# rueberger/MJHMC

Hardware: AMD Instinct MI355X
Metric: particle-steps/sec (ndims x nparticles x L) (higher is better)
Workload: dtype f64 state (ProductOfT: around the f32 matrix-core force)

## Files before the change

### mjhmc_amd/csrc/dense_pot64_kernels.hpp

```cpp
#pragma once
#ifndef __HIPCC_RTC__
#include <hip/hip_runtime.h>
#endif
#include <stdint.h>

#include "dense_pot.hpp"
#include "dense_pot_tile.hpp"
#include "group_form.hpp"

namespace mjhmc {

template <int NB>
struct DVecN;
template <>
struct DVecN<1> {
  using type = double;
};
template <>
struct DVecN<2> {
  using type = __attribute__((ext_vector_type(2))) double;
};
template <>
struct DVecN<4> {
  using type = __attribute__((ext_vector_type(4))) double;
};
template <int NB>
__device__ __forceinline__ double dget(const typename DVecN<NB>::type& v, int r) {
  if constexpr (NB == 1) return v;
  else return v[r];
}
template <int NB>
__device__ __forceinline__ void dset(typename DVecN<NB>::type& v, int r, double x) {
  if constexpr (NB == 1) v = x;
  else v[r] = x;
}

template <int NB>
__device__ __forceinline__ int q_off(int q) { return NB * ((q & 3) + 8 * (q >> 2)); }
template <int NB>
__device__ __forceinline__ const double* lane_row(const double* base, int64_t p, int w, int h) {
  return base + (size_t)p * (128 * NB) + 32 * NB * w + 4 * NB * h;
}
template <int NB>
__device__ __forceinline__ double* lane_row(double* base, int64_t p, int w, int h) {
  return base + (size_t)p * (128 * NB) + 32 * NB * w + 4 * NB * h;
}
template <int NB>
__device__ __forceinline__ typename DVecN<NB>::type dv_load(const double* lrow, int q) {
  return *reinterpret_cast<const typename DVecN<NB>::type*>(lrow + q_off<NB>(q));
}
template <int NB>
__device__ __forceinline__ void dv_store(double* lrow, int q, const typename DVecN<NB>::type& v) {
  *reinterpret_cast<typename DVecN<NB>::type*>(lrow + q_off<NB>(q)) = v;
}

template <int NB>
constexpr int kA64 = NB == 4 ? 8 : 16;
template <int NB>
using AReg64 = AReg<NB, kA64<NB>>;

constexpr int kPark = 8;
template <int NB>
struct Shared64 {
  Shared<NB> s;
  double red64[4][kP];
  double zn[128 * NB];
  f32x4 park[kPark / 2][256];
};

using uvec4 = __attribute__((ext_vector_type(4))) unsigned;
using f64x2 = __attribute__((ext_vector_type(2))) double;

template <int NB>
struct PieceOf {
  using type = uvec4;
};
template <>
struct PieceOf<1> {
  using type = unsigned long long;
};
__device__ __forceinline__ int here(int lane_const) {
  asm volatile("" : "+v"(lane_const));
  return lane_const;
}
template <int NB>
struct Stage {
  using P = typename PieceOf<NB>::type;
  static constexpr int PB = sizeof(P);
  static constexpr int RB = 1024 * NB;
  static constexpr int RP = RB / PB;
  static constexpr int K = 32 * RP / 256;
  static constexpr int KB = K < 16 ? K : 16;
};
__device__ __forceinline__ unsigned stage_addr(int row, int piece, int pb, int rb) {
  return (unsigned)(row * rb + ((piece ^ (row & 15)) * pb));
}
template <int NB>
__device__ __forceinline__ void stage_rows_in(const double* rows, int64_t p, char* img) {
  using S = Stage<NB>;
  using P = typename S::P;
  const int t = here(threadIdx.x);
#pragma unroll 1
  for (int i0 = 0; i0 < S::K; i0 += S::KB) {
    P buf[S::KB];
#pragma unroll
    for (int i = 0; i < S::KB; ++i) {
      const int k = (i0 + i) * 256 + t, row = k / S::RP, piece = k % S::RP;
      const int64_t pr = __shfl((long long)p, row);
      buf[i] = *reinterpret_cast<const P*>(reinterpret_cast<const char*>(rows) + (size_t)pr * S::RB + (size_t)piece * S::PB);
    }
#pragma unroll
    for (int i = 0; i < S::KB; ++i) {
      const int k = (i0 + i) * 256 + t, row = k / S::RP, piece = k % S::RP;
      *reinterpret_cast<P*>(img + stage_addr(row, piece, S::PB, S::RB)) = buf[i];
    }
  }
}
template <int NB>
__device__ __forceinline__ void stage_rows_out(double* rows, int64_t p, const char* img) {
  using S = Stage<NB>;
  using P = typename S::P;
  const int t = here(threadIdx.x);
#pragma unroll 1
  for (int i0 = 0; i0 < S::K; i0 += S::KB) {
#pragma unroll
    for (int i = 0; i < S::KB; ++i) {
      const int k = (i0 + i) * 256 + t, row = k / S::RP, piece = k % S::RP;
      const int64_t pr = __shfl((long long)p, row);
      *reinterpret_cast<P*>(reinterpret_cast<char*>(rows) + (size_t)pr * S::RB + (size_t)piece * S::PB) =
          *reinterpret_cast<const P*>(img + stage_addr(row, piece, S::PB, S::RB));
    }
  }
}
template <int NB>
__device__ __forceinline__ typename DVecN<NB>::type stage_get(const char* img, int w, int c, int h, int q) {
  using S = Stage<NB>;
  const int first = (8 * NB * (32 * w + acc_row(q, h))) / S::PB;
  if constexpr (NB == 4) {
    const f64x2 lo = *reinterpret_cast<const f64x2*>(img + stage_addr(c, first, S::PB, S::RB));
    const f64x2 hi = *reinterpret_cast<const f64x2*>(img + stage_addr(c, first + 1, S::PB, S::RB));
    typename DVecN<4>::type v;
    v[0] = lo[0];
    v[1] = lo[1];
    v[2] = hi[0];
    v[3] = hi[1];
    return v;
  } else {
    return *reinterpret_cast<const typename DVecN<NB>::type*>(img + stage_addr(c, first, S::PB, S::RB));
  }
}
template <int NB>
__device__ __forceinline__ void stage_put(char* img, int w, int c, int h, int q, const typename DVecN<NB>::type& v) {
  using S = Stage<NB>;
  const int first = (8 * NB * (32 * w + acc_row(q, h))) / S::PB;
  if constexpr (NB == 4) {
    f64x2 lo, hi;
    lo[0] = v[0];
    lo[1] = v[1];
    hi[0] = v[2];
    hi[1] = v[3];
    *reinterpret_cast<f64x2*>(img + stage_addr(c, first, S::PB, S::RB)) = lo;
    *reinterpret_cast<f64x2*>(img + stage_addr(c, first + 1, S::PB, S::RB)) = hi;
  } else {
    *reinterpret_cast<typename DVecN<NB>::type*>(img + stage_addr(c, first, S::PB, S::RB)) = v;
  }
}
template <int NB>
__device__ __forceinline__ char* stage_image(Shared<NB>& s) {
  static_assert(sizeof(s.pub) == 32 * Stage<NB>::RB, "the staging image is the two B-operand images");
  return reinterpret_cast<char*>(&s.pub[0][0]);
}

template <int NB>
struct VTile {
  double b[NB][16];
};

template <int NB, int NKICK>
__device__ __forceinline__ void kick_drift_pass(const Tile<NB>& g, VTile<NB>& v, VTile<NB>& x, double c, double eps,
                                                PubWave<NB>* pub0, int w, int lane) {
#pragma unroll
  for (int q4 = 0; q4 < 4; ++q4) {
    f32x4 px[NB];
#pragma unroll
    for (int qq = 0; qq < 4; ++qq) {
      const int q = 4 * q4 + qq;
#pragma unroll
      for (int r = 0; r < NB; ++r) {
        const double t = c * (double)g.b[r][q];
        double vv = v.b[r][q];
        vv = vv + t;
        if constexpr (NKICK == 2) vv = vv + t;
        v.b[r][q] = vv;
        const double xx = x.b[r][q] + eps * vv;
        x.b[r][q] = xx;
        px[r][qq] = (float)xx;
      }
    }
#pragma unroll
    for (int r = 0; r < NB; ++r) pub0[w].v[r][q4][lane] = px[r];
    __builtin_amdgcn_sched_barrier(0);
  }
}

template <int NB>
__device__ __forceinline__ double closing_kick(const Tile<NB>& g, VTile<NB>& v, double c) {
  double s = 0.0;
#pragma unroll
  for (int q = 0; q < 16; ++q)
#pragma unroll
    for (int r = 0; r < NB; ++r) {
      const double vv = v.b[r][q] + c * (double)g.b[r][q];
      v.b[r][q] = vv;
      s = s + vv * vv;
    }
  return s;
}

template <int NB, class SH>
__device__ __forceinline__ double column_sum(SH& sh, int w, int c, int h, double part) {
  const double both = swap32_sum(part);
  if (h == 0) sh.red64[w][c] = both;
  __syncthreads();
  const double tot = sh.red64[0][c] + sh.red64[1][c] + sh.red64[2][c] + sh.red64[3][c];
  __syncthreads();
  return tot;
}

template <int NB>
__device__ __forceinline__ void staged_start(Shared<NB>& s, const double* xin, const double* vin, const double* gin, int64_t p,
                                             int w, int c, int h, Tile<NB>& g, VTile<NB>& v, VTile<NB>& x, bool neg) {
  char* img = stage_image<NB>(s);
  c = here(c), w = here(w), h = here(h);
  stage_rows_in<NB>(xin, p, img);
  __syncthreads();
#pragma unroll
  for (int q = 0; q < 16; ++q) {
    const typename DVecN<NB>::type xx = stage_get<NB>(img, w, c, h, q);
#pragma unroll
    for (int r = 0; r < NB; ++r) x.b[r][q] = dget<NB>(xx, r);
  }
  __syncthreads();
  stage_rows_in<NB>(gin, p, img);
  __syncthreads();
#pragma unroll
  for (int q = 0; q < 16; ++q) {
    const typename DVecN<NB>::type gg = stage_get<NB>(img, w, c, h, q);
#pragma unroll
    for (int r = 0; r < NB; ++r) g.b[r][q] = (float)dget<NB>(gg, r);
  }
  __syncthreads();
  stage_rows_in<NB>(vin, p, img);
  __syncthreads();
#pragma unroll
  for (int q = 0; q < 16; ++q) {
    const typename DVecN<NB>::type vv = stage_get<NB>(img, w, c, h, q);
#pragma unroll
    for (int r = 0; r < NB; ++r) v.b[r][q] = neg ? -dget<NB>(vv, r) : dget<NB>(vv, r);
  }
  __syncthreads();
}

template <int NB>
__device__ __forceinline__ void staged_end_x(Shared<NB>& s, double* xout, int64_t p, int w, int c, int h, const VTile<NB>& x) {
  char* img = stage_image<NB>(s);
  c = here(c), w = here(w), h = here(h);
#pragma unroll
  for (int q = 0; q < 16; ++q) {
    typename DVecN<NB>::type xx;
#pragma unroll
    for (int r = 0; r < NB; ++r) dset<NB>(xx, r, x.b[r][q]);
    stage_put<NB>(img, w, c, h, q, xx);
  }
  __syncthreads();
  stage_rows_out<NB>(xout, p, img);
  __syncthreads();
}
template <int NB>
__device__ __forceinline__ void staged_end_vg(Shared<NB>& s, double* vout, double* gout, int64_t p, int w, int c, int h,
                                              const VTile<NB>& v, const Tile<NB>& g) {
  using DV = typename DVecN<NB>::type;
  char* img = stage_image<NB>(s);
  c = here(c), w = here(w), h = here(h);
#pragma unroll
  for (int q = 0; q < 16; ++q) {
    DV vv;
#pragma unroll
    for (int r = 0; r < NB; ++r) dset<NB>(vv, r, v.b[r][q]);
    stage_put<NB>(img, w, c, h, q, vv);
  }
  __syncthreads();
  stage_rows_out<NB>(vout, p, img);
  __syncthreads();
#pragma unroll
  for (int q = 0; q < 16; ++q) {
    DV gg;
#pragma unroll
    for (int r = 0; r < NB; ++r) dset<NB>(gg, r, (double)g.b[r][q]);
    stage_put<NB>(img, w, c, h, q, gg);
  }
  __syncthreads();
  stage_rows_out<NB>(gout, p, img);
  __syncthreads();
}

template <int NB, class XP>
__device__ __forceinline__ double pot64_trajectory(const PotModel& mdl, const XP& xp, AReg64<NB>& ar, Shared64<NB>& sh, int w, int c, int h,
                                                   int lane, Tile<NB>& g, VTile<NB>& v, VTile<NB>& x, int L, double eps,
                                                   double chalf, float* ex) {
  PubWave<NB>* pub0 = sh.s.pub[0];
  kick_drift_pass<NB, 1>(g, v, x, chalf, eps, pub0, w, lane);
  for (int s = 0; s < L; ++s) {
    [[maybe_unused]] const int stamp_slot = s;
    POT_STAMP(0);
    if constexpr (NB == 4) {
#pragma unroll
      for (int k = 0; k < kPark / 2; ++k) {
        f64x2 two;
        two[0] = v.b[NB - 1][15 - 2 * k];
        two[1] = v.b[NB - 1][14 - 2 * k];
        sh.park[k][threadIdx.x] = __builtin_bit_cast(f32x4, two);
      }
    }
    pot_gradient_published<NB>(mdl, xp, ar, sh.s, w, c, h, lane, g, s == L - 1, ex, s);
    if constexpr (NB == 4) {
#pragma unroll
      for (int k = 0; k < kPark / 2; ++k) {
        const f64x2 two = __builtin_bit_cast(f64x2, sh.park[k][threadIdx.x]);
        v.b[NB - 1][15 - 2 * k] = two[0];
        v.b[NB - 1][14 - 2 * k] = two[1];
      }
#pragma unroll
      for (int r = 0; r < NB; ++r)
#pragma unroll
        for (int q = 0; q < 16; ++q) use_here(v.b[r][q]);
    }
    POT_STAMP(6);
    if (s < L - 1) kick_drift_pass<NB, 2>(g, v, x, chalf, eps, pub0, w, lane);
    POT_STAMP(7);
  }
  const double part = closing_kick<NB>(g, v, chalf);
  return column_sum<NB>(sh, w, c, h, part) / 2.0;
}


template <int NB>
struct Finish64Shared {
  struct {
    int move[kP];
  } s;
  double red64[4][kP];
  double zn[128 * NB];
};

template <int NB, bool REPLAY, int MODE, bool FIX, class SH>
__device__ __forceinline__ void pot64_finish(const Pot64JumpArgs& a, SH& sh, int64_t p, bool alive, size_t roff, int w, int c,
                                             int h, const VTile<NB>& v, const Tile<NB>& g) {
  using DV = typename DVecN<NB>::type;
  const double* xin = a.X_in + roff;
  const double* vin = a.V_in + roff;
  const double* gin = a.G_in + roff;
  double* xo = a.X_out + roff;
  double* vo = a.V_out + roff;
  double* go = a.G_out + roff;
  const int mv = sh.s.move[c];
  const int k = mv & 3;
  bool take, flip, refresh;
  if constexpr (MODE == kModeControl) {
    const bool accept = k & 1, fl = k & 2;
    take = accept;
    flip = accept != fl;
    refresh = (mv & 4) != 0;
  } else {
    take = k == 0;
    flip = (MODE == kModeCT && k == 0) || k == 1;
    refresh = k == 2;
  }
  const bool tile_refreshes = __ballot(refresh) != 0ull;
  if (!FIX || !take) {
#pragma unroll
    for (int q = 0; q < 16; ++q) {
      DV gg;
      if (take) {
        if constexpr (!FIX) {
          DV vv;
#pragma unroll
          for (int r = 0; r < NB; ++r) {
            dset<NB>(vv, r, flip ? -v.b[r][q] : v.b[r][q]);
            dset<NB>(gg, r, (double)g.b[r][q]);
          }
          dv_store<NB>(vo, q, vv);
        }
      } else {
        gg = dv_load<NB>(gin, q);
        dv_store<NB>(xo, q, dv_load<NB>(xin, q));
      }
      dv_store<NB>(go, q, gg);
    }
  }
  double s2 = 0.0;
  if (!take || (REPLAY && refresh)) {
    const double* vsrc = take ? (const double*)vo : vin;
    const bool fl2 = flip && !take;
    const double* nrow = REPLAY ? lane_row<NB>(a.noise, alive ? p : 0, w, h) : nullptr;
#pragma unroll 1
    for (int q = 0; q < 16; ++q) {
      DV vv = dv_load<NB>(vsrc, q);
      if (fl2) vv = -vv;
      if constexpr (REPLAY) {
        if (refresh) {
          const DV z = dv_load<NB>(nrow, q);
#pragma unroll
          for (int r = 0; r < NB; ++r) {
            const double t = dget<NB>(vv, r) * a.r_keep + dget<NB>(z, r) * a.r_mix;
            dset<NB>(vv, r, t);
            s2 = s2 + t * t;
          }
        }
      }
      dv_store<NB>(vo, q, vv);
    }
  }
  if constexpr (!REPLAY) {
    unsigned cols = (unsigned)(__ballot(refresh) & 0xFFFFFFFFull);
    while (cols) {
      const int c0 = __ffs((int)cols) - 1;
      cols &= cols - 1;
      const int64_t p0 = __shfl((long long)p, c0);
      column_normals<NB, double>(a.key, (uint32_t)(a.first_pid + (p0 < a.N ? p0 : 0)), a.D, sh.zn);
      __syncthreads();
      if (c == c0) {
        const double* zrow = sh.zn + 32 * NB * w + 4 * NB * h;
#pragma unroll 1
        for (int q = 0; q < 16; ++q) {
          DV vv = dv_load<NB>(vo, q);
          const DV z = *reinterpret_cast<const DV*>(zrow + q_off<NB>(q));
#pragma unroll
          for (int r = 0; r < NB; ++r) {
            const double t = dget<NB>(vv, r) * a.r_keep + dget<NB>(z, r) * a.r_mix;
            dset<NB>(vv, r, t);
            s2 = s2 + t * t;
          }
          dv_store<NB>(vo, q, vv);
        }
      }
      __syncthreads();
    }
  }
  if (tile_refreshes) {
    const double evr = column_sum<NB>(sh, w, c, h, s2) / 2.0;
    if (refresh && w == 0 && h == 0) a.EV_out[p] = evr;
  }
}

template <bool REPLAY, int MODE>
__device__ __forceinline__ int pot64_decide(const Pot64JumpArgs& a, double H0, double HL, double Hflf, int64_t pp, uint32_t pid,
                                            double& best, bool& bad, bool& gate) {
  JumpArgs<double> ja;
  ja.p_r = a.p_r;
  ja.p_flip = a.p_flip;
  ja.rexp = a.rexp;
  ja.runif = a.runif;
  ja.N = a.N;
  const LaneMap m = LaneMap::one_lane();
  int k = 0;
  if constexpr (MODE == kModeMJHMC) {
    decide<double, REPLAY>(ja, a.key, m, H0, HL, Hflf, pp, pid, k, best, bad);
  } else if constexpr (MODE == kModeCT) {
    decide_ct<double, REPLAY>(ja, a.key, m, H0, HL, pp, pid, k, best, bad);
  } else {
    double uacc, uflip, ugate;
    if constexpr (REPLAY) {
      uacc = a.runif[pp];
      uflip = a.runif[a.N + pp];
      ugate = a.runif[2 * a.N];
    } else {
      const u32x4 q = philox4x32_10(pid, a.key.tick_lo, a.key.tick_hi, kSlotExpR, a.key.k0, a.key.k1);
      const u32x4 f = philox4x32_10(pid, a.key.tick_lo, a.key.tick_hi, kSlotFlip, a.key.k0, a.key.k1);
      const u32x4 gq = philox4x32_10(0xFFFFFFFFu, a.key.tick_lo, a.key.tick_hi, kSlotFlip, a.key.k0, a.key.k1);
      uacc = u53(q.w2, q.w3);
      uflip = u53(f.w0, f.w1);
      ugate = u53(gq.w2, gq.w3);
    }
    const double dH = H0 - HL;
    const bool accept = !(dH < 0.0) || (uacc < exp(dH));
    const bool flip = uflip < a.p_flip;
    gate = ugate < a.p_r;
    k = (accept ? 1 : 0) | (flip ? 2 : 0);
  }
  return k;
}


}
```

### mjhmc_amd/csrc/dense_pot_tile.hpp

```cpp
#pragma once
#ifndef __HIPCC_RTC__
#include <hip/hip_runtime.h>
#endif
#include <stdint.h>

#include "dense_pot.hpp"
#include "timing_variants.hpp"

namespace mjhmc {

using f32x16 = __attribute__((ext_vector_type(16))) float;
using f32x4 = __attribute__((ext_vector_type(4))) float;

constexpr int kP = 32;

__device__ __forceinline__ int acc_row(int q, int h) { return (q & 3) + 8 * (q >> 2) + 4 * h; }

template <int NB>
struct Tile {
  f32x16 b[NB];
};

template <int NB>
struct VecN;
template <>
struct VecN<1> {
  using type = float;
};
template <>
struct VecN<2> {
  using type = __attribute__((ext_vector_type(2))) float;
};
template <>
struct VecN<4> {
  using type = f32x4;
};

template <int NB>
__device__ __forceinline__ float vget(const typename VecN<NB>::type& v, int r) {
  if constexpr (NB == 1) return v;
  else return v[r];
}
template <int NB>
__device__ __forceinline__ void vset(typename VecN<NB>::type& v, int r, float x) {
  if constexpr (NB == 1) v = x;
  else v[r] = x;
}

template <int NB>
__device__ __forceinline__ void tile_load(const float* base, int64_t p, int w, int h, Tile<NB>& t) {
  using V = typename VecN<NB>::type;
  const float* row = base + (size_t)p * (128 * NB) + 32 * NB * w;
#pragma unroll
  for (int q = 0; q < 16; ++q) {
    const V v = *reinterpret_cast<const V*>(row + NB * acc_row(q, h));
#pragma unroll
    for (int r = 0; r < NB; ++r) t.b[r][q] = vget<NB>(v, r);
  }
}

template <int NB>
__device__ __forceinline__ void tile_store(float* base, int64_t p, int w, int h, const Tile<NB>& t) {
  using V = typename VecN<NB>::type;
  float* row = base + (size_t)p * (128 * NB) + 32 * NB * w;
#pragma unroll
  for (int q = 0; q < 16; ++q) {
    V v;
#pragma unroll
    for (int r = 0; r < NB; ++r) vset<NB>(v, r, t.b[r][q]);
    *reinterpret_cast<V*>(row + NB * acc_row(q, h)) = v;
  }
}

template <int NB>
struct PubWave {
  f32x4 v[NB][4][64];
};

template <int NB>
__device__ __forceinline__ void publish(PubWave<NB>& dst, int lane, const Tile<NB>& t) {
#pragma unroll
  for (int r = 0; r < NB; ++r)
#pragma unroll
    for (int q4 = 0; q4 < 4; ++q4) {
      f32x4 v;
      v[0] = t.b[r][4 * q4 + 0];
      v[1] = t.b[r][4 * q4 + 1];
      v[2] = t.b[r][4 * q4 + 2];
      v[3] = t.b[r][4 * q4 + 3];
      dst.v[r][q4][lane] = v;
    }
}

template <int NB, int AQ = 16>
__device__ __forceinline__ void a_chunk_load(const float* mlane, int chunk, typename VecN<NB>::type (&dst)[AQ]) {
  using V = typename VecN<NB>::type;
  constexpr int DIM = 128 * NB;
  const float* base = mlane + (size_t)(32 * NB * (chunk / NB) + (chunk % NB)) * DIM;
#pragma unroll
  for (int q = 0; q < AQ; ++q) dst[q] = *reinterpret_cast<const V*>(base + (size_t)(NB * ((q & 3) + 8 * (q >> 2))) * DIM);
}

template <int NB>
__device__ __forceinline__ typename VecN<NB>::type buf_load(__amdgpu_buffer_rsrc_t r, unsigned voff, unsigned soff) {
  using V = typename VecN<NB>::type;
  if constexpr (NB == 4) return __builtin_bit_cast(V, __builtin_amdgcn_raw_buffer_load_b128(r, voff, soff, 0));
  else if constexpr (NB == 2) return __builtin_bit_cast(V, __builtin_amdgcn_raw_buffer_load_b64(r, voff, soff, 0));
  else return __builtin_bit_cast(V, __builtin_amdgcn_raw_buffer_load_b32(r, voff, soff, 0));
}
template <int NB>
__device__ __forceinline__ __amdgpu_buffer_rsrc_t a_rsrc(const float* M) {
  constexpr int DIM = 128 * NB;
  return __builtin_amdgcn_make_buffer_rsrc((void*)M, 0, DIM * DIM * 4, 0x00020000);
}
template <int NB>
__device__ __forceinline__ void a_chunk_load_buf(__amdgpu_buffer_rsrc_t r, unsigned lane_bytes, int chunk,
                                                 typename VecN<NB>::type (&dst)[16]) {
  constexpr int DIM = 128 * NB;
  const unsigned cbase = (unsigned)(32 * NB * (chunk / NB) + (chunk % NB)) * (unsigned)(DIM * 4);
#pragma unroll
  for (int q = 0; q < 16; ++q) dst[q] = buf_load<NB>(r, lane_bytes, cbase + (unsigned)(NB * ((q & 3) + 8 * (q >> 2)) * DIM * 4));
}

template <int NB>
__device__ __forceinline__ void chunk_mfma(const f32x4* bbase, int chunk, int lane, const typename VecN<NB>::type (&a)[16],
                                           f32x4& bnext, Tile<NB>& acc) {
  constexpr int NG = 16 * NB;
#pragma unroll
  for (int q4 = 0; q4 < 4; ++q4) {
    const f32x4 b4 = bnext;
    const int t = 4 * chunk + q4 + 1;
    bnext = bbase[(size_t)(t < NG ? t : NG - 1) * 64 + lane];
    __builtin_amdgcn_sched_barrier(0);
#pragma unroll
    for (int qq = 0; qq < 4; ++qq) {
#pragma unroll
      for (int r = 0; r < NB; ++r)
        acc.b[r] = __builtin_amdgcn_mfma_f32_32x32x2f32(vget<NB>(a[4 * q4 + qq], r), b4[qq], acc.b[r], 0, 0, 0);
    }
    __builtin_amdgcn_sched_barrier(0);
  }
}

template <int NB>
__device__ __forceinline__ void chunk_mfma_ld(const f32x4* bbase, int chunk, int lane, const typename VecN<NB>::type (&a)[16],
                                              f32x4& bnext, Tile<NB>& acc, __amdgpu_buffer_rsrc_t rs, unsigned lane_bytes,
                                              unsigned cbase, typename VecN<NB>::type (&aload)[16]) {
  constexpr int NG = 16 * NB, DIM = 128 * NB;
#pragma unroll
  for (int q4 = 0; q4 < 4; ++q4) {
    const f32x4 b4 = bnext;
    const int t = 4 * chunk + q4 + 1;
    bnext = bbase[(size_t)(t < NG ? t : NG - 1) * 64 + lane];
    __builtin_amdgcn_sched_barrier(0);
#pragma unroll
    for (int qq = 0; qq < 4; ++qq) {
      const int q = 4 * q4 + qq;
#pragma unroll
      for (int r = 0; r < NB; ++r)
        acc.b[r] = __builtin_amdgcn_mfma_f32_32x32x2f32(vget<NB>(a[q], r), b4[qq], acc.b[r], 0, 0, 0);
      aload[q] = buf_load<NB>(rs, lane_bytes, cbase + (unsigned)(NB * ((q & 3) + 8 * (q >> 2)) * DIM * 4));
      __builtin_amdgcn_sched_barrier(0);
    }
    __builtin_amdgcn_sched_barrier(0);
  }
}

template <int NB>
__device__ __forceinline__ void gemm_dim(const float* __restrict__ M, const float* __restrict__ Mnext, const PubWave<NB>* pub,
                                         int w, int c, int h, int lane, typename VecN<NB>::type (&a0)[16], Tile<NB>& acc) {
  constexpr int DIM = 128 * NB, NCH = 4 * NB;
  const size_t lane_off = (size_t)(4 * NB * h) * DIM + 32 * NB * w + NB * c;
  const unsigned lane_bytes = (unsigned)(lane_off * sizeof(float));
  const __amdgpu_buffer_rsrc_t rM = a_rsrc<NB>(M), rN = a_rsrc<NB>(Mnext);
  const f32x4* bbase = &pub[0].v[0][0][0];
  typename VecN<NB>::type a1[16];
  f32x4 bnext = bbase[lane];
#pragma unroll 1
  for (int chunk = 0; chunk < NCH; chunk += 2) {
    const bool more = chunk + 2 < NCH;
    const int c1 = chunk + 1, c2 = more ? chunk + 2 : 0;
    chunk_mfma_ld<NB>(bbase, chunk, lane, a0, bnext, acc, rM, lane_bytes,
                      (unsigned)(32 * NB * (c1 / NB) + (c1 % NB)) * (unsigned)(DIM * 4), a1);
    chunk_mfma_ld<NB>(bbase, chunk + 1, lane, a1, bnext, acc, more ? rM : rN, lane_bytes,
                      (unsigned)(32 * NB * (c2 / NB) + (c2 % NB)) * (unsigned)(DIM * 4), a0);
  }
}

template <int NB, int HALF, int NHALF>
__device__ __forceinline__ void half_mfma_ld(const f32x4* bbase, int chunk, int lane, const typename VecN<NB>::type (&a)[8],
                                             f32x4& bnext, Tile<NB>& acc, __amdgpu_buffer_rsrc_t rs, unsigned lane_bytes,
                                             unsigned cbase, typename VecN<NB>::type (&aload)[8]) {
  constexpr int NG = 16 * NB, DIM = 128 * NB;
#pragma unroll
  for (int q4 = 2 * HALF; q4 < 2 * HALF + 2; ++q4) {
    const f32x4 b4 = bnext;
    const int t = 4 * chunk + q4 + 1;
    bnext = bbase[(size_t)(t < NG ? t : NG - 1) * 64 + lane];
    __builtin_amdgcn_sched_barrier(0);
#pragma unroll
    for (int qq = 0; qq < 4; ++qq) {
      const int j = 4 * (q4 - 2 * HALF) + qq, qn = 8 * NHALF + j;
#pragma unroll
      for (int r = 0; r < NB; ++r)
        acc.b[r] = __builtin_amdgcn_mfma_f32_32x32x2f32(vget<NB>(a[j], r), b4[qq], acc.b[r], 0, 0, 0);
      aload[j] = buf_load<NB>(rs, lane_bytes, cbase + (unsigned)(NB * ((qn & 3) + 8 * (qn >> 2)) * DIM * 4));
      __builtin_amdgcn_sched_barrier(0);
    }
    __builtin_amdgcn_sched_barrier(0);
  }
}

template <int NB>
__device__ __forceinline__ void gemm_dim_half(const float* __restrict__ M, const float* __restrict__ Mnext, const PubWave<NB>* pub,
                                              int w, int c, int h, int lane, typename VecN<NB>::type (&a0)[8], Tile<NB>& acc) {
  constexpr int DIM = 128 * NB, NCH = 4 * NB;
  const size_t lane_off = (size_t)(4 * NB * h) * DIM + 32 * NB * w + NB * c;
  const unsigned lane_bytes = (unsigned)(lane_off * sizeof(float));
  const __amdgpu_buffer_rsrc_t rM = a_rsrc<NB>(M), rN = a_rsrc<NB>(Mnext);
  const f32x4* bbase = &pub[0].v[0][0][0];
  typename VecN<NB>::type a1[8];
  f32x4 bnext = bbase[lane];
  auto cbase_of = [](int ch) { return (unsigned)(32 * NB * (ch / NB) + (ch % NB)) * (unsigned)(DIM * 4); };
#pragma unroll 1
  for (int chunk = 0; chunk < NCH; chunk += 2) {
    const bool more = chunk + 2 < NCH;
    const int c1 = chunk + 1, c2 = more ? chunk + 2 : 0;
    half_mfma_ld<NB, 0, 1>(bbase, chunk, lane, a0, bnext, acc, rM, lane_bytes, cbase_of(chunk), a1);
    half_mfma_ld<NB, 1, 0>(bbase, chunk, lane, a1, bnext, acc, rM, lane_bytes, cbase_of(c1), a0);
    half_mfma_ld<NB, 0, 1>(bbase, c1, lane, a0, bnext, acc, rM, lane_bytes, cbase_of(c1), a1);
    half_mfma_ld<NB, 1, 0>(bbase, c1, lane, a1, bnext, acc, more ? rM : rN, lane_bytes, cbase_of(c2), a0);
  }
}

template <int NB, int AQ = 16>
struct AReg {
  typename VecN<NB>::type a0[AQ];
};
template <int AQ>
struct AReg<1, AQ> {
  float w1[4][16];
  float w2[4][16];
};

template <int NB, int AQ>
__device__ __forceinline__ void areg_load(const PotModel& mdl, int w, int c, int h, AReg<NB, AQ>& ar) {
  if constexpr (NB == 1) {
    const float* m1 = mdl.W1 + (size_t)(4 * h) * 128 + 32 * w + c;
    const float* m2 = mdl.W2T + (size_t)(4 * h) * 128 + 32 * w + c;
#pragma unroll
    for (int chunk = 0; chunk < 4; ++chunk) {
      a_chunk_load<1>(m1, chunk, ar.w1[chunk]);
      a_chunk_load<1>(m2, chunk, ar.w2[chunk]);
    }
  } else {
    a_chunk_load<NB, AQ>(mdl.W1 + (size_t)(4 * NB * h) * (128 * NB) + 32 * NB * w + NB * c, 0, ar.a0);
  }
}

template <int NB, bool SECOND, int AQ>
__device__ __forceinline__ void gemm_any(const PotModel& mdl, AReg<NB, AQ>& ar, const PubWave<NB>* pub, int w, int c,
                                         int h, int lane, Tile<NB>& acc) {
  if constexpr (NB == 1) {
    const int kdim = mdl.ndims;
#pragma unroll
    for (int chunk = 0; chunk < 4; ++chunk) {
      const float(&a)[16] = SECOND ? ar.w2[chunk] : ar.w1[chunk];
      const f32x4(*blk)[64] = pub[chunk].v[0];
#pragma unroll
      for (int q4 = 0; q4 < 4; ++q4) {
        if (32 * chunk + 8 * q4 < kdim) {
          const f32x4 b4 = blk[q4][lane];
#pragma unroll
          for (int qq = 0; qq < 4; ++qq)
            acc.b[0] = __builtin_amdgcn_mfma_f32_32x32x2f32(a[4 * q4 + qq], b4[qq], acc.b[0], 0, 0, 0);
        }
      }
    }
  } else if constexpr (AQ == 8) {
    gemm_dim_half<NB>(SECOND ? mdl.W2T : mdl.W1, SECOND ? mdl.W1 : mdl.W2T, pub, w, c, h, lane, ar.a0, acc);
  } else {
    gemm_dim<NB>(SECOND ? mdl.W2T : mdl.W1, SECOND ? mdl.W1 : mdl.W2T, pub, w, c, h, lane, ar.a0, acc);
  }
}

template <int NB>
__device__ __forceinline__ void rowvec_load(const float* vec, int w, int h, Tile<NB>& t) {
  using V = typename VecN<NB>::type;
  const float* base = vec + 32 * NB * w;
#pragma unroll
  for (int q = 0; q < 16; ++q) {
    const V v = *reinterpret_cast<const V*>(base + NB * acc_row(q, h));
#pragma unroll
    for (int r = 0; r < NB; ++r) t.b[r][q] = vget<NB>(v, r);
  }
}

__device__ __forceinline__ float half_sum(float s) {
  const auto sw = __builtin_amdgcn_permlane32_swap(__float_as_int(s), __float_as_int(s), false, false);
  return __int_as_float(sw[0]) + __int_as_float(sw[1]);
}

template <int NB>
struct Shared {
  PubWave<NB> pub[2][4];
  float red[2][4][kP];
  int move[kP];
  float cb[128 * NB];
  float zn[128 * NB];
};

template <int NB>
struct FinishShared {
  float red[2][4][kP];
  int move[kP];
  float zn[128 * NB];
};

template <int NB, typename F>
__device__ __forceinline__ void column_normals(const RngKey& key, uint32_t pid, int D, F* zn) {
  const int pair = threadIdx.x;
  if (pair < 64 * NB) {
    double z0, z1;
    normal_pair(key, pid, (uint32_t)pair, z0, z1);
    zn[2 * pair] = 2 * pair < D ? (F)z0 : (F)0;
    zn[2 * pair + 1] = 2 * pair + 1 < D ? (F)z1 : (F)0;
  }
}

template <int NB>
__device__ __forceinline__ void stage_bias(const PotModel& mdl, Shared<NB>& sh) {
  for (int i = threadIdx.x; i < 128 * NB; i += 256) sh.cb[i] = mdl.cb[i];
}


struct PotExperts {
  static constexpr bool kProductOfT = true;
};

template <int NB, class XP, int AQ>
__device__ __forceinline__ void pot_gradient_published(const PotModel& mdl, const XP& xp, AReg<NB, AQ>& ar, Shared<NB>& sh, int w, int c, int h,
                                                       int lane, Tile<NB>& g, bool want_energy, float* energy_out,
                                                       int stamp_slot = 0) {
  __syncthreads();
  POT_STAMP(1);
  Tile<NB> u;
  rowvec_load<NB>(sh.cb, w, h, u);
  gemm_any<NB, false>(mdl, ar, sh.pub[0], w, c, h, lane, u);
  POT_STAMP(2);
  if constexpr (XP::kProductOfT) {
    if (want_energy) {
      using V = typename VecN<NB>::type;
      const float* al = mdl.alpha + 32 * NB * w;
      float s = 0.f;
#pragma unroll
      for (int q = 0; q < 16; ++q) {
        const V a4 = *reinterpret_cast<const V*>(al + NB * acc_row(q, h));
#pragma unroll
        for (int r = 0; r < NB; ++r) s += vget<NB>(a4, r) * logf(1.0f + u.b[r][q] * u.b[r][q]);
      }
      const float part = half_sum(s);
      if (h == 0) sh.red[0][w][c] = part;
    }
#pragma unroll
    for (int r = 0; r < NB; ++r)
#pragma unroll
      for (int q = 0; q < 16; ++q) {
        const float uu = u.b[r][q];
        u.b[r][q] = uu * __builtin_amdgcn_rcpf(1.0f + uu * uu);
      }
  } else {
    if (want_energy) {
      const float part = half_sum(xp.template energy_sum<NB>(u, w, h));
      if (h == 0) sh.red[0][w][c] = part;
    }
    xp.template phi<NB>(u, w, h);
  }
  publish<NB>(sh.pub[1][w], lane, u);
  POT_STAMP(3);
  __syncthreads();
  POT_STAMP(4);
#pragma unroll
  for (int r = 0; r < NB; ++r)
#pragma unroll
    for (int q = 0; q < 16; ++q) g.b[r][q] = 0.f;
  gemm_any<NB, true>(mdl, ar, sh.pub[1], w, c, h, lane, g);
  POT_STAMP(5);
  if (want_energy && energy_out) {
    *energy_out = sh.red[0][0][c] + sh.red[0][1][c] + sh.red[0][2][c] + sh.red[0][3][c];
  }
}

template <int NB, class XP>
__device__ __forceinline__ void pot_gradient(const PotModel& mdl, const XP& xp, AReg<NB>& ar, Shared<NB>& sh, int w, int c, int h,
                                             int lane, const Tile<NB>& x, Tile<NB>& g, bool want_energy,
                                             float* energy_out) {
  [[maybe_unused]] const int stamp_slot = 0;
  POT_STAMP(0);
  publish<NB>(sh.pub[0][w], lane, x);
  pot_gradient_published<NB>(mdl, xp, ar, sh, w, c, h, lane, g, want_energy, energy_out);
}

template <int NB, class SH>
__device__ __forceinline__ float pot_kinetic(SH& sh, int w, int c, int h, const Tile<NB>& v) {
  float s = 0.f;
#pragma unroll
  for (int r = 0; r < NB; ++r)
#pragma unroll
    for (int q = 0; q < 16; ++q) s += v.b[r][q] * v.b[r][q];
  const float part = half_sum(s);
  if (h == 0) sh.red[1][w][c] = part;
  __syncthreads();
  const float tot = (sh.red[1][0][c] + sh.red[1][1][c] + sh.red[1][2][c] + sh.red[1][3][c]) / 2.0f;
  __syncthreads();
  return tot;
}

template <int NB, class XP>
__device__ __forceinline__ void pot_trajectory(const PotModel& mdl, const XP& xp, AReg<NB>& ar, Shared<NB>& sh, int w, int c, int h,
                                               int lane, Tile<NB>& x, Tile<NB>& v, Tile<NB>& g, int L, float eps,
                                               float chalf, float* ex) {
  if (L > 0) {
#pragma unroll
    for (int r = 0; r < NB; ++r)
#pragma unroll
      for (int q = 0; q < 16; ++q) v.b[r][q] = v.b[r][q] + chalf * g.b[r][q];
  }
  for (int s = 0; s < L; ++s) {
#pragma unroll
    for (int r = 0; r < NB; ++r)
#pragma unroll
      for (int q = 0; q < 16; ++q) x.b[r][q] = x.b[r][q] + eps * v.b[r][q];
    pot_gradient<NB>(mdl, xp, ar, sh, w, c, h, lane, x, g, s == L - 1, ex);
    const float ck = s == L - 1 ? chalf : 2.0f * chalf;
#pragma unroll
    for (int r = 0; r < NB; ++r)
#pragma unroll
      for (int q = 0; q < 16; ++q) v.b[r][q] = v.b[r][q] + ck * g.b[r][q];
  }
}

template <int NB>
__device__ __forceinline__ void pot_normals(const RngKey& key, uint32_t pid, int w, int h, int D, Tile<NB>& z) {
#pragma unroll 1
  for (int q = 0; q < 16; ++q) {
    const int d = 32 * NB * w + NB * acc_row(q, h);
    double zz[4] = {0, 0, 0, 0};
    normal_pair(key, pid, (uint32_t)(d >> 1), zz[0], zz[1]);
    if constexpr (NB == 4) normal_pair(key, pid, (uint32_t)((d >> 1) + 1), zz[2], zz[3]);
    if constexpr (NB == 1) {
      z.b[0][q] = d < D ? (float)((d & 1) ? zz[1] : zz[0]) : 0.f;
    } else {
#pragma unroll
      for (int r = 0; r < NB; ++r) z.b[r][q] = d + r < D ? (float)zz[r] : 0.f;
    }
  }
}

}
```

Before: 63.23 billion.

## Interleave phi and kick-drift epilogue work into the last MFMA chunk of each GEMM

Adds a tail variant of the half-GEMM loop whose final chunk interleaves dependent VALU work between MFMAs, for the NB=4 ProductOfT path. In the first GEMM, the phi transform and its shared-memory publish for finished accumulator blocks are done inside the MFMA shadow. In the second GEMM, part of the next step's kick-drift update and its publish are done the same way. The kick-drift pass and the phi epilogue then skip the slices already handled. The aim is to hide epilogue VALU and LDS-store latency behind matrix-core work, at the cost of more register pressure and more complex, scheduling-sensitive code.

```diff
diff --git a/mjhmc_amd/csrc/dense_pot64_kernels.hpp b/mjhmc_amd/csrc/dense_pot64_kernels.hpp
--- a/mjhmc_amd/csrc/dense_pot64_kernels.hpp
+++ b/mjhmc_amd/csrc/dense_pot64_kernels.hpp
@@ -176,7 +176,7 @@
   double b[NB][16];
 };
 
-template <int NB, int NKICK>
+template <int NB, int NKICK, int DONE = 0>
 __device__ __forceinline__ void kick_drift_pass(const Tile<NB>& g, VTile<NB>& v, VTile<NB>& x, double c, double eps,
                                                 PubWave<NB>* pub0, int w, int lane) {
 #pragma unroll
@@ -187,6 +187,7 @@
       const int q = 4 * q4 + qq;
 #pragma unroll
       for (int r = 0; r < NB; ++r) {
+        if (r < NB - 1 && q < DONE) continue;
         const double t = c * (double)g.b[r][q];
         double vv = v.b[r][q];
         vv = vv + t;
@@ -198,10 +199,44 @@
       }
     }
 #pragma unroll
-    for (int r = 0; r < NB; ++r) pub0[w].v[r][q4][lane] = px[r];
+    for (int r = 0; r < NB; ++r)
+      if (!(r < NB - 1 && 4 * q4 < DONE)) pub0[w].v[r][q4][lane] = px[r];
     __builtin_amdgcn_sched_barrier(0);
   }
 }
+
+template <bool B>
+struct Flag {
+  static constexpr bool value = B;
+};
+
+template <int NB>
+struct StepTail {
+  static constexpr bool kOn = true, kFill = true;
+  static constexpr int kPhi = 1, kPass = 1;
+  static constexpr int kDone = 8 * kPass;
+  VTile<NB>& v;
+  VTile<NB>& x;
+  double c, eps;
+  PubWave<NB>& pubw;
+  int lane;
+  f32x4& px;
+  __device__ __forceinline__ void pass_slice(const Tile<NB>& g, int rb, int j) const {
+#pragma unroll
+    for (int e = 0; e < kPass; ++e) {
+      const int q = kPass * j + e;
+      const double t = c * (double)g.b[rb][q];
+      double vv = v.b[rb][q];
+      vv = vv + t;
+      vv = vv + t;
+      v.b[rb][q] = vv;
+      const double xx = x.b[rb][q] + eps * vv;
+      x.b[rb][q] = xx;
+      px[q & 3] = (float)xx;
+      if ((q & 3) == 3) pubw.v[rb][q >> 2][lane] = px;
+    }
+  }
+};
 
 template <int NB>
 __device__ __forceinline__ double closing_kick(const Tile<NB>& g, VTile<NB>& v, double c) {
@@ -309,11 +344,11 @@
                                                    int lane, Tile<NB>& g, VTile<NB>& v, VTile<NB>& x, int L, double eps,
                                                    double chalf, float* ex) {
   PubWave<NB>* pub0 = sh.s.pub[0];
+  constexpr bool kTail = XP::kProductOfT && NB == 4 && kA64<NB> == 8;
   kick_drift_pass<NB, 1>(g, v, x, chalf, eps, pub0, w, lane);
-  for (int s = 0; s < L; ++s) {
-    [[maybe_unused]] const int stamp_slot = s;
-    POT_STAMP(0);
-    if constexpr (NB == 4) {
+  if constexpr (kTail) {
+    auto gradient = [&](auto tail, [[maybe_unused]] int stamp_slot) {
+      POT_STAMP(0);
 #pragma unroll
       for (int k = 0; k < kPark / 2; ++k) {
         f64x2 two;
@@ -321,9 +356,13 @@
         two[1] = v.b[NB - 1][14 - 2 * k];
         sh.park[k][threadIdx.x] = __builtin_bit_cast(f32x4, two);
       }
-    }
-    pot_gradient_published<NB>(mdl, xp, ar, sh.s, w, c, h, lane, g, s == L - 1, ex, s);
-    if constexpr (NB == 4) {
+      if constexpr (decltype(tail)::value) {
+        f32x4 px;
+        pot_gradient_published<NB>(mdl, xp, ar, sh.s, w, c, h, lane, g, false, ex, stamp_slot,
+                                   StepTail<NB>{v, x, chalf, eps, pub0[w], lane, px});
+      } else {
+        pot_gradient_published<NB>(mdl, xp, ar, sh.s, w, c, h, lane, g, true, ex, stamp_slot, BlockTail());
+      }
 #pragma unroll
       for (int k = 0; k < kPark / 2; ++k) {
         const f64x2 two = __builtin_bit_cast(f64x2, sh.park[k][threadIdx.x]);
@@ -334,10 +373,45 @@
       for (int r = 0; r < NB; ++r)
 #pragma unroll
         for (int q = 0; q < 16; ++q) use_here(v.b[r][q]);
+      POT_STAMP(6);
+    };
+    for (int s = 0; s < L - 1; ++s) {
+      gradient(Flag<true>{}, s);
+      kick_drift_pass<NB, 2, StepTail<NB>::kDone>(g, v, x, chalf, eps, pub0, w, lane);
+      [[maybe_unused]] const int stamp_slot = s;
+      POT_STAMP(7);
+    }
+    gradient(Flag<false>{}, L - 1);
+  } else {
+  for (int s = 0; s < L; ++s) {
+    [[maybe_unused]] const int stamp_slot = s;
+    POT_STAMP(0);
+    if constexpr (NB == 4) {
+#pragma unroll
+      for (int k = 0; k < kPark / 2; ++k) {
+        f64x2 two;
+        two[0] = v.b[NB - 1][15 - 2 * k];
+        two[1] = v.b[NB - 1][14 - 2 * k];
+        sh.park[k][threadIdx.x] = __builtin_bit_cast(f32x4, two);
+      }
+    }
+    pot_gradient_published<NB>(mdl, xp, ar, sh.s, w, c, h, lane, g, s == L - 1, ex, s);
+    if constexpr (NB == 4) {
+#pragma unroll
+      for (int k = 0; k < kPark / 2; ++k) {
+        const f64x2 two = __builtin_bit_cast(f64x2, sh.park[k][threadIdx.x]);
+        v.b[NB - 1][15 - 2 * k] = two[0];
+        v.b[NB - 1][14 - 2 * k] = two[1];
+      }
+#pragma unroll
+      for (int r = 0; r < NB; ++r)
+#pragma unroll
+        for (int q = 0; q < 16; ++q) use_here(v.b[r][q]);
     }
     POT_STAMP(6);
     if (s < L - 1) kick_drift_pass<NB, 2>(g, v, x, chalf, eps, pub0, w, lane);
     POT_STAMP(7);
+  }
   }
   const double part = closing_kick<NB>(g, v, chalf);
   return column_sum<NB>(sh, w, c, h, part) / 2.0;
diff --git a/mjhmc_amd/csrc/dense_pot_tile.hpp b/mjhmc_amd/csrc/dense_pot_tile.hpp
--- a/mjhmc_amd/csrc/dense_pot_tile.hpp
+++ b/mjhmc_amd/csrc/dense_pot_tile.hpp
@@ -233,6 +233,58 @@
   }
 }
 
+template <int NB, class Fill>
+__device__ __forceinline__ void half_mfma_tail(const f32x4* bbase, int chunk, int lane, const typename VecN<NB>::type (&a)[8],
+                                               const f32x4 bfirst, Tile<NB>& acc, __amdgpu_buffer_rsrc_t rs, unsigned lane_bytes,
+                                               unsigned cbase, typename VecN<NB>::type (&aload)[8], Fill&& fill) {
+  constexpr int DIM = 128 * NB;
+  static_assert(NB == 4, "one A request per four MFMAs fills the next half-set in exactly 8 NB MFMAs at NB = 4");
+  const f32x4 bq[2] = {bfirst, bbase[(size_t)(4 * chunk + 3) * 64 + lane]};
+  __builtin_amdgcn_sched_barrier(0);
+#pragma unroll
+  for (int r = 0; r < NB; ++r) {
+#pragma unroll
+    for (int j = 0; j < 8; ++j) {
+      acc.b[r] = __builtin_amdgcn_mfma_f32_32x32x2f32(vget<NB>(a[j], r), bq[j >> 2][j & 3], acc.b[r], 0, 0, 0);
+      if ((j & 3) == 0) {
+        const int qn = 2 * r + (j >> 2);
+        aload[qn] = buf_load<NB>(rs, lane_bytes, cbase + (unsigned)(NB * ((qn & 3) + 8 * (qn >> 2)) * DIM * 4));
+      }
+      __builtin_amdgcn_sched_barrier(0);
+      if (r > 0) {
+        fill(r - 1, j);
+        __builtin_amdgcn_sched_barrier(0);
+      }
+    }
+  }
+}
+
+template <int NB, class Fill>
+__device__ __forceinline__ void gemm_dim_half_tail(const float* __restrict__ M, const float* __restrict__ Mnext, const PubWave<NB>* pub,
+                                                   int w, int c, int h, int lane, typename VecN<NB>::type (&a0)[8], Tile<NB>& acc,
+                                                   Fill&& fill) {
+  constexpr int DIM = 128 * NB, NCH = 4 * NB;
+  const size_t lane_off = (size_t)(4 * NB * h) * DIM + 32 * NB * w + NB * c;
+  const unsigned lane_bytes = (unsigned)(lane_off * sizeof(float));
+  const __amdgpu_buffer_rsrc_t rM = a_rsrc<NB>(M), rN = a_rsrc<NB>(Mnext);
+  const f32x4* bbase = &pub[0].v[0][0][0];
+  typename VecN<NB>::type a1[8];
+  f32x4 bnext = bbase[lane];
+  auto cbase_of = [](int ch) { return (unsigned)(32 * NB * (ch / NB) + (ch % NB)) * (unsigned)(DIM * 4); };
+#pragma unroll 1
+  for (int chunk = 0; chunk < NCH - 2; chunk += 2) {
+    const int c1 = chunk + 1, c2 = chunk + 2;
+    half_mfma_ld<NB, 0, 1>(bbase, chunk, lane, a0, bnext, acc, rM, lane_bytes, cbase_of(chunk), a1);
+    half_mfma_ld<NB, 1, 0>(bbase, chunk, lane, a1, bnext, acc, rM, lane_bytes, cbase_of(c1), a0);
+    half_mfma_ld<NB, 0, 1>(bbase, c1, lane, a0, bnext, acc, rM, lane_bytes, cbase_of(c1), a1);
+    half_mfma_ld<NB, 1, 0>(bbase, c1, lane, a1, bnext, acc, rM, lane_bytes, cbase_of(c2), a0);
+  }
+  half_mfma_ld<NB, 0, 1>(bbase, NCH - 2, lane, a0, bnext, acc, rM, lane_bytes, cbase_of(NCH - 2), a1);
+  half_mfma_ld<NB, 1, 0>(bbase, NCH - 2, lane, a1, bnext, acc, rM, lane_bytes, cbase_of(NCH - 1), a0);
+  half_mfma_ld<NB, 0, 1>(bbase, NCH - 1, lane, a0, bnext, acc, rM, lane_bytes, cbase_of(NCH - 1), a1);
+  half_mfma_tail<NB>(bbase, NCH - 1, lane, a1, bnext, acc, rN, lane_bytes, cbase_of(0), a0, fill);
+}
+
 template <int NB, int AQ = 16>
 struct AReg {
   typename VecN<NB>::type a0[AQ];
@@ -338,45 +390,93 @@
   static constexpr bool kProductOfT = true;
 };
 
-template <int NB, class XP, int AQ>
+struct NoTail {
+  static constexpr bool kOn = false, kFill = false;
+};
+struct BlockTail {
+  static constexpr bool kOn = true, kFill = false;
+};
+
+template <int NB, class XP, int AQ, class TL = NoTail>
 __device__ __forceinline__ void pot_gradient_published(const PotModel& mdl, const XP& xp, AReg<NB, AQ>& ar, Shared<NB>& sh, int w, int c, int h,
                                                        int lane, Tile<NB>& g, bool want_energy, float* energy_out,
-                                                       int stamp_slot = 0) {
+                                                       int stamp_slot = 0, TL tl = TL()) {
+  constexpr bool kTail = TL::kOn && XP::kProductOfT && NB == 4 && AQ == 8;
+  constexpr bool kFill = kTail && TL::kFill;
   __syncthreads();
   POT_STAMP(1);
   Tile<NB> u;
   rowvec_load<NB>(sh.cb, w, h, u);
-  gemm_any<NB, false>(mdl, ar, sh.pub[0], w, c, h, lane, u);
+  if constexpr (kTail) {
+    [[maybe_unused]] f32x4 hq;
+    gemm_dim_half_tail<NB>(mdl.W1, mdl.W2T, sh.pub[0], w, c, h, lane, ar.a0, u, [&]([[maybe_unused]] int rb, [[maybe_unused]] int j) {
+      if constexpr (kFill) {
+#pragma unroll
+        for (int e = 0; e < TL::kPhi; ++e) {
+          const int q = TL::kPhi * j + e;
+          float uu = u.b[rb][q];
+          asm volatile("" : "+v"(uu));
+          hq[q & 3] = uu * __builtin_amdgcn_rcpf(1.0f + uu * uu);
+          if ((q & 3) == 3) sh.pub[1][w].v[rb][q >> 2][lane] = hq;
+        }
+      }
+    });
+  } else {
+    gemm_any<NB, false>(mdl, ar, sh.pub[0], w, c, h, lane, u);
+  }
   POT_STAMP(2);
-  if constexpr (XP::kProductOfT) {
-    if (want_energy) {
-      using V = typename VecN<NB>::type;
-      const float* al = mdl.alpha + 32 * NB * w;
-      float s = 0.f;
-#pragma unroll
-      for (int q = 0; q < 16; ++q) {
-        const V a4 = *reinterpret_cast<const V*>(al + NB * acc_row(q, h));
-#pragma unroll
-        for (int r = 0; r < NB; ++r) s += vget<NB>(a4, r) * logf(1.0f + u.b[r][q] * u.b[r][q]);
-      }
-      const float part = half_sum(s);
-      if (h == 0) sh.red[0][w][c] = part;
-    }
+  if constexpr (kFill) {
+    static_assert(TL::kPhi == 1 || TL::kPhi == 2, "whole quads of a block per eight gaps");
+    constexpr int DONE = 8 * TL::kPhi;
 #pragma unroll
     for (int r = 0; r < NB; ++r)
 #pragma unroll
-      for (int q = 0; q < 16; ++q) {
-        const float uu = u.b[r][q];
-        u.b[r][q] = uu * __builtin_amdgcn_rcpf(1.0f + uu * uu);
+      for (int q4 = (r < NB - 1 ? DONE / 4 : 0); q4 < 4; ++q4) {
+        f32x4 v4;
+#pragma unroll
+        for (int qq = 0; qq < 4; ++qq) {
+          const float uu = u.b[r][4 * q4 + qq];
+          v4[qq] = uu * __builtin_amdgcn_rcpf(1.0f + uu * uu);
+        }
+        sh.pub[1][w].v[r][q4][lane] = v4;
       }
   } else {
-    if (want_energy) {
-      const float part = half_sum(xp.template energy_sum<NB>(u, w, h));
-      if (h == 0) sh.red[0][w][c] = part;
-    }
-    xp.template phi<NB>(u, w, h);
-  }
-  publish<NB>(sh.pub[1][w], lane, u);
+    if constexpr (XP::kProductOfT) {
+      if (want_energy) {
+        using V = typename VecN<NB>::type;
+        int we = w, he = h, ce = c;
+        if constexpr (kTail) {
+          asm volatile("" : "+v"(we));
+          asm volatile("" : "+v"(he));
+          asm volatile("" : "+v"(ce));
+        }
+        const float* al = mdl.alpha + 32 * NB * we;
+        float s = 0.f;
+#pragma unroll
+        for (int q = 0; q < 16; ++q) {
+          const V a4 = *reinterpret_cast<const V*>(al + NB * acc_row(q, he));
+#pragma unroll
+          for (int r = 0; r < NB; ++r) s += vget<NB>(a4, r) * logf(1.0f + u.b[r][q] * u.b[r][q]);
+        }
+        const float part = half_sum(s);
+        if (he == 0) sh.red[0][we][ce] = part;
+      }
+#pragma unroll
+      for (int r = 0; r < NB; ++r)
+#pragma unroll
+        for (int q = 0; q < 16; ++q) {
+          const float uu = u.b[r][q];
+          u.b[r][q] = uu * __builtin_amdgcn_rcpf(1.0f + uu * uu);
+        }
+    } else {
+      if (want_energy) {
+        const float part = half_sum(xp.template energy_sum<NB>(u, w, h));
+        if (h == 0) sh.red[0][w][c] = part;
+      }
+      xp.template phi<NB>(u, w, h);
+    }
+    publish<NB>(sh.pub[1][w], lane, u);
+  }
   POT_STAMP(3);
   __syncthreads();
   POT_STAMP(4);
@@ -384,7 +484,13 @@
   for (int r = 0; r < NB; ++r)
 #pragma unroll
     for (int q = 0; q < 16; ++q) g.b[r][q] = 0.f;
-  gemm_any<NB, true>(mdl, ar, sh.pub[1], w, c, h, lane, g);
+  if constexpr (kTail) {
+    gemm_dim_half_tail<NB>(mdl.W2T, mdl.W1, sh.pub[1], w, c, h, lane, ar.a0, g, [&]([[maybe_unused]] int rb, [[maybe_unused]] int j) {
+      if constexpr (kFill) tl.pass_slice(g, rb, j);
+    });
+  } else {
+    gemm_any<NB, true>(mdl, ar, sh.pub[1], w, c, h, lane, g);
+  }
   POT_STAMP(5);
   if (want_energy && energy_out) {
     *energy_out = sh.red[0][0][c] + sh.red[0][1][c] + sh.red[0][2][c] + sh.red[0][3][c];
```

Result: faster. 64.16 billion, median of 6 (+1.5%).
